# gopi-erabati/Object-Pose-Estimation

Measured on AMD Instinct MI355X. Metric: ICP iterations/sec (1M scene pts vs 100k model pts) at 1/2/4/8 GPU, higher is better.
Workload: dtype f32

## Files before the change

### object-pose-estimation_amd/csrc/api.hip

```cpp
#include <algorithm>
#include <cfloat>
#include <cmath>
#include <cstring>
#include <limits>
#include <numeric>

#include <chrono>
#include <thread>

#include "ope_internal.hpp"
#include "stage_host.hpp"

namespace ope {

static thread_local std::string g_global_err;

constexpr double kGridMaxTreeShare = 0.03, kGridMinTreeShare = 0.015;
constexpr size_t kGridMinQueries = 0;
constexpr float kHeavyLoadFactor = 1.0f;
constexpr float kHeavyLoadFactorStatic = 1.5f;
constexpr float kHeavyMaxChunksPerWave = 1.8f;

int set_err(ope_ctx *ctx, int code, const std::string &msg) {
  if (ctx) ctx->err = msg;
// ... 179 lines not shown
  if (ctx->grid_auto && grid_probe_poll(ctx, it_done) > 0) {
    const int rcs = switch_kernel(ctx, true, it_done, nch);
    if (rcs != OPE_OK) return rcs;
    --ctx->acc_launches;
    return enqueue_accumulate(ctx, atomic_sums);
  }
  if (ctx->plan_pending) {
    OPE_HIP(ctx, hipStreamWaitEvent(ctx->stream, ctx->ev_plan_done, 0));
    ctx->plan_cur ^= 1;
    ctx->plan_cur_slots = ctx->plan_pending_slots;
    ctx->plan_valid = true;
    ctx->plan_pending = false;
  }
  const bool plan_step = !no_plan && nch > 1 && it_done >= 1 && plan_step_after(ctx, it_done);
  if (plan_step) {
    const float chunks_per_wave = (float)nch / (float)(ctx->n_cu * 4 * kAccWavesPerSimd);
    const float heavy_factor = chunks_per_wave > kHeavyMaxChunksPerWave ? 0.0f : std::min(7.0f, std::max(2.0f, 1.2f + 1.5f * chunks_per_wave));
    const bool static_deal = ctx->cert_run && ctx->cert_seen && ctx->run_params.corr_mode == OPE_CORR_NEAREST && !ctx->run_params.use_reciprocal;
    const float load_factor = chunks_per_wave > kHeavyMaxChunksPerWave ? (static_deal ? kHeavyLoadFactorStatic : kHeavyLoadFactor) : 0.0f;
    hipStream_t ps = ctx->plan_stream;
    const int nxt = ctx->plan_cur ^ 1;
    OPE_HIP(ctx, hipEventRecord(ctx->ev_acc_done, ctx->stream));
    OPE_HIP(ctx, hipStreamWaitEvent(ps, ctx->ev_acc_done, 0));
    if (ctx->grid_auto && it_done >= 8) {
      const int rcp = grid_probe_issue(ctx, ps);
      if (rcp != OPE_OK) return rcp;
    }
    size_t tb = ctx->plan_tmp_bytes;
    if (chunk_plan(ps, cost_r, ctx->d_plan_sorted[nxt], ctx->d_chunk_ids, ctx->d_plan_order[nxt], nch, ctx->d_plan_tmp, tb) != 0)
      return set_err(ctx, OPE_EHIP, "chunk plan sort failed");
    uint32_t *out = ctx->d_plan_out + 8 * nxt;
    const uint32_t group_slots = static_deal ? 8u : (uint32_t)kFrontLanes;
    const float slot_share = static_deal ? kOctSlotShare : kFrontSlotShare;
    plan_heavy(ps, ctx->d_plan_sorted[nxt], nch, heavy_factor, load_factor, (uint32_t)ctx->acc_blocks * (kAccBlock / 64), group_slots, slot_share, out);
    const bool slots = ctx->run_params.corr_mode == OPE_CORR_NEAREST && !ctx->run_params.use_reciprocal;
    if (slots) plan_slots(ps, ctx->d_plan_sorted[nxt], nch, out, group_slots, slot_share, ctx->d_plan_slots[nxt]);
    OPE_HIP(ctx, hipEventRecord(ctx->ev_plan_done, ps));
    ctx->plan_pending = true;
    ctx->plan_pending_slots = slots;
  }
  const ope_icp_params &p = ctx->run_params;
  const bool nrm = p.corr_mode == OPE_CORR_NORMAL_SHOOTING || p.use_surface_normal_rej || p.use_self_occluded_rej ||
                   p.estimator == OPE_EST_POINT_TO_PLANE_LLS;
  const bool recip = p.use_reciprocal != 0;
  const uint32_t packet_min = (uint32_t)ctx->n_cu * 4u * (uint32_t)kAccWavesPerSimd;
  const bool packet = p.tree_walk == OPE_WALK_PACKET ? (ctx->run_tgt->d_axis2 != nullptr && p.corr_mode == OPE_CORR_NEAREST && !recip)
                      : p.tree_walk == OPE_WALK_LANE ? false : nch > packet_min;
  ++ctx->kernel_launches[p.corr_mode != OPE_CORR_NEAREST ? OPE_KERNEL_KNN : (packet && !recip) ? OPE_KERNEL_TREE_PACKET : OPE_KERNEL_TREE_LANE];
  const bool certify = ctx->cert_run && ctx->cert_seen && p.corr_mode == OPE_CORR_NEAREST && !recip;
  AccTreeLaunch a;
  fill_acc_launch(ctx, a, certify, cost_w, atomic_sums);
  a.nrm = nrm;
  a.chunk_order = ctx->plan_valid ? ctx->d_plan_order[ctx->plan_cur] : nullptr;
  a.mode = p.corr_mode;
  a.recip = recip;
  a.srcix = recip ? ctx->run_src_index->view() : ctx->run_tgt->view();
  a.work_counter = ctx->d_work_counter;
  a.packet = packet;
  a.k_normal_shooting = p.k_normal_shooting;
  a.slot_list = (ctx->plan_valid && ctx->plan_cur_slots) ? ctx->d_plan_slots[ctx->plan_cur] : nullptr;
  a.knn_rk = p.corr_mode == OPE_CORR_NORMAL_SHOOTING ? ctx->d_knn_rk : nullptr;
  a.plan_out = ctx->d_plan_out + 8 * ctx->plan_cur;
  a.deal = ctx->d_deal;
  a.deal_parity = ctx->deal_parity;
  launch_icp_accumulate(a);
  ctx->deal_parity ^= 1u;
  return OPE_OK;
// ... 1397 lines not shown
```

### object-pose-estimation_amd/csrc/icp_kernels.hip

```cpp
#include <cstdlib>
#include <hip/hip_ext.h>

#include "bvh_traverse.hpp"
#include "lm_solve.hpp"
#include "icp_update.hpp"

namespace ope {

typedef const __attribute__((address_space(3))) float *lds_cfloat_ptr;
static_assert(kCertCand >= 1 && kCertCand <= 8, "skip certificates: candidates per query");

__device__ __forceinline__ uint32_t chain_load(const uint32_t *p) { return __hip_atomic_load(p, __ATOMIC_RELAXED, __HIP_MEMORY_SCOPE_AGENT); }
__device__ __forceinline__ void chain_store(uint32_t *p, uint32_t v) { __hip_atomic_store(p, v, __ATOMIC_RELAXED, __HIP_MEMORY_SCOPE_AGENT); }
__device__ __forceinline__ void chain_wait_own_memory_ops() { __builtin_amdgcn_s_waitcnt(0); }
__device__ __forceinline__ bool acc_launch_begin(const IcpState *st, uint32_t *chain, uint32_t chain_seq, float *s_const, uint32_t wait_ticks) {
  if (chain == nullptr) return st->done == 0;
  __shared__ uint32_t s_go[2];
  if (threadIdx.x == 0) {
    uint32_t go = 1u;
    const unsigned long long t0 = wall_clock64();
    while ((int32_t)(chain_load(chain + 1) - chain_seq) < 0) {
      if (wall_clock64() - t0 > (unsigned long long)wait_ticks) { go = 0u; atomicOr(chain + 2, 1u); break; }
      __builtin_amdgcn_s_sleep(2);
    }
    s_go[0] = go;
  }
  __syncthreads();
  if (threadIdx.x < 12) s_const[threadIdx.x] = __hip_atomic_load(&st->Ff[threadIdx.x], __ATOMIC_RELAXED, __HIP_MEMORY_SCOPE_AGENT);
  else if (threadIdx.x == 12) s_go[1] = (uint32_t)__hip_atomic_load(&st->done, __ATOMIC_RELAXED, __HIP_MEMORY_SCOPE_AGENT);
  else if (threadIdx.x == 17) s_const[17] = __hip_atomic_load(&st->last_move, __ATOMIC_RELAXED, __HIP_MEMORY_SCOPE_AGENT);
  __syncthreads();
  return s_go[0] != 0u && s_go[1] == 0u;
}
__device__ __forceinline__ void acc_launch_end(uint32_t *chain) {
  if (chain == nullptr) return;
  chain_wait_own_memory_ops();
  __syncthreads();
  if (threadIdx.x == 0) __hip_atomic_fetch_add(chain, 1u, __ATOMIC_RELAXED, __HIP_MEMORY_SCOPE_AGENT);
}

__device__ __forceinline__ uint32_t deal_pop(uint32_t *counters, uint32_t stripe, uint32_t lane_id) {
  uint32_t k = 0u;
  if (lane_id == 0u) k = __hip_atomic_fetch_add(counters + stripe * kDealLineWords, 1u, __ATOMIC_RELAXED, __HIP_MEMORY_SCOPE_AGENT);
  return k;
}
constexpr uint32_t kDealNone = 0xffffffffu;
__device__ __forceinline__ uint32_t deal_next(uint32_t k, uint32_t stripe, uint32_t n_stripes, uint32_t n_waves, uint32_t n_slots) {
  const uint32_t slot = n_waves + stripe + k * n_stripes;
  return slot < n_slots ? slot : kDealNone;
}
__device__ __forceinline__ void deal_clear_other_set(uint32_t *deal, uint32_t parity) {
  if (blockIdx.x == 0 && threadIdx.x < kDealStripes)
    __hip_atomic_store(deal + (size_t)(parity ^ 1u) * kDealStripes * kDealLineWords + threadIdx.x * kDealLineWords, 0u, __ATOMIC_RELAXED, __HIP_MEMORY_SCOPE_AGENT);
}

template <bool NRM>
__device__ __forceinline__ void add_query_sums(double *acc, lds_cfloat_ptr cs2, uint32_t lane_id, bool ok, bool p2p, float x, float y, float z,
                                               const float4 t, const float4 tn, float d2) {
    {
      asm volatile("" : "+v"(cs2));
      const float psx = cs2[12], psy = cs2[13], psz = cs2[14];
      const double sx = (double)x - (double)psx, sy = (double)y - (double)psy, sz = (double)z - (double)psz;
      const double tx = (double)t.x - (double)psx, ty = (double)t.y - (double)psy, tz = (double)t.z - (double)psz;
      const double w = ok ? 1.0 : 0.0;
      double term[kNumSums];
      term[0] = w;
      term[1] = w * sx; term[2] = w * sy; term[3] = w * sz;
      term[4] = w * tx; term[5] = w * ty; term[6] = w * tz;
      term[7] = w * (tx * sx); term[8] = w * (tx * sy); term[9] = w * (tx * sz);
      term[10] = w * (ty * sx); term[11] = w * (ty * sy); term[12] = w * (ty * sz);
      term[13] = w * (tz * sx); term[14] = w * (tz * sy); term[15] = w * (tz * sz);
      term[16] = ok ? (double)d2 : 0.0;
#pragma unroll
      for (int k = 0; k < kNumSums; ++k) {
        const double r = row16_sum(term[k]);
        if ((lane_id & 15u) == 0u) unsafeAtomicAdd(acc + k, r);
      }
      if (NRM && p2p) {
        const float v0 = __fsub_rn(__fmul_rn(tn.z, y), __fmul_rn(tn.y, z));
        const float v1 = __fsub_rn(__fmul_rn(tn.x, z), __fmul_rn(tn.z, x));
        const float v2 = __fsub_rn(__fmul_rn(tn.y, x), __fmul_rn(tn.x, y));
        const float dd = __fsub_rn(__fsub_rn(__fsub_rn(__fadd_rn(__fadd_rn(__fmul_rn(tn.x, t.x), __fmul_rn(tn.y, t.y)), __fmul_rn(tn.z, t.z)),
                                                         __fmul_rn(tn.x, x)), __fmul_rn(tn.y, y)), __fmul_rn(tn.z, z));
        const double v[6] = {w * (double)v0, w * (double)v1, w * (double)v2, w * (double)tn.x, w * (double)tn.y, w * (double)tn.z};
        int slot = kNumSums;
#pragma unroll
// ... 113 lines not shown
  else if (threadIdx.x < 15) s_const[threadIdx.x] = (float)st->pivot[threadIdx.x - 12];
  else if (threadIdx.x == 15) s_const[15] = best0;
  else if (threadIdx.x == 17) { if (chain == nullptr) s_const[17] = st->last_move; }
  else if (threadIdx.x == 30) s_ncert = 0u;
  __syncthreads();
  if (MODE == 2 && knn_rk != nullptr && blockIdx.x == 0 && threadIdx.x == 0) const_cast<IcpState *>(st)->knn_acc_flag = 1;
  constexpr bool cert_on = CERT;
  if (cert_on && threadIdx.x == 0) {
    s_const[18] = st->cert_k;
    s_const[19] = st->cert_cap;
    if (blockIdx.x == 0) atomicAdd(work_counter + 42, 1u);
  }
  if (cert_on) __syncthreads();
  const bool rej_sn = NRM && st->use_surface_normal_rej;
  const bool rej_so = NRM && st->use_self_occluded_rej;
  const bool store_pos = st->estimator == OPE_EST_POINT_TO_PLANE_LM;
  const double thr_sn = st->surface_normal_thr, thr_so = st->self_occluded_thr;
  const double max_dist_unsq = st->max_corr_dist;
  const int kk = st->k_normal_shooting;

  if ((threadIdx.x & 63u) < (uint32_t)kNumSumsMax) s_red[threadIdx.x >> 6][threadIdx.x & 63u] = 0.0;
  const bool p2p = NRM && st->estimator == OPE_EST_POINT_TO_PLANE_LLS;

  const uint32_t lane_id = threadIdx.x & 63u;
  const uint32_t n_waves = gridDim.x * (BLOCK / 64);
  const uint32_t wave_id = (uint32_t)__builtin_amdgcn_readfirstlane((int)(blockIdx.x * (BLOCK / 64) + (threadIdx.x >> 6)));
  const uint32_t n_chunks = (src.n_valid + 63u) / 64u;
  const bool measuring = chunk_order && measuring_launch != 0u;
  const uint32_t n_heavy = (OCT_OK && chunk_order && !measuring) ? min(plan_out[0], n_chunks) : 0u;
  constexpr uint32_t GW = CERT ? 8u : (uint32_t)kFrontLanes;
  const bool listed = OCT_OK && slot_list != nullptr && chunk_order != nullptr && !measuring && n_heavy > 0u && plan_out[6] == GW;
  const uint32_t n_slots = n_chunks + (GW - 1u) * n_heavy;
  const bool dealt = chunk_order != nullptr && !CERT;
  uint32_t *const deal_set = deal + (size_t)deal_parity * kDealStripes * kDealLineWords;
  const uint32_t n_stripes = min(kDealStripes, n_waves);
  const uint32_t stripe = wave_id % n_stripes;
  const uint32_t n_alone = (dealt || !chunk_order) ? 0u
                           : listed             ? min(plan_out[7], n_waves / 2u)
                                                : min(min(plan_out[5] + (measuring ? min(plan_out[0], n_chunks) : 0u), n_chunks - n_heavy), n_waves / 2u);
  const uint32_t n_snake = n_slots - n_alone, snake_waves = n_waves - n_alone;
  auto static_slot = [&](uint32_t r) -> uint32_t {
    if (wave_id < n_alone) return r == 0u ? (listed ? wave_id : GW * n_heavy + wave_id) : kDealNone;
    const uint32_t w = wave_id - n_alone;
    const uint32_t sn = r * snake_waves + ((r & 1u) ? (snake_waves - 1u - w) : w);
    if (sn >= n_snake) return kDealNone;
    return (listed || sn >= GW * n_heavy) ? sn + n_alone : sn;
  };
  uint32_t round = 0u;
  uint32_t slot = static_slot(0u);
  while (slot != kDealNone) {
    uint32_t ticket_v = 0u;
    bool oct;
    uint32_t ord, sub;
    if (listed) {
      const uint32_t e = slot_list[slot];
      oct = (e >> 31) != 0u;
      sub = (e >> 28) & 7u;
      ord = e & 0x0fffffffu;
    } else {
      oct = slot < GW * n_heavy;
      ord = oct ? (slot / GW) : (n_heavy + (slot - GW * n_heavy));
      sub = slot % GW;
    }
    const uint32_t chunk = chunk_order ? chunk_order[ord] : ord;
    const uint32_t base = chunk * 64u;
    const unsigned long long t_begin = __builtin_amdgcn_s_memtime();
    const uint32_t i = oct ? (base + sub * (64u / GW) + (lane_id / GW)) : (base + lane_id);
    const bool active = i < src.n_valid;
    const bool owner = active && (!oct || (lane_id & (GW - 1u)) == 0u);
    lds_cfloat_ptr cst = (lds_cfloat_ptr)s_const;
    asm volatile("" : "+v"(cst));
    float F[12];
#pragma unroll
    for (int k = 0; k < 12; ++k) F[k] = cst[k];
    const float4 s = src.xyzw[active ? i : base];
    const float x = xform_row(F + 0, s.x, s.y, s.z);
    const float y = xform_row(F + 4, s.x, s.y, s.z);
    const float z = xform_row(F + 8, s.x, s.y, s.z);
    float nx = 0.f, ny = 0.f, nz = 0.f;
    if (NRM && src.nrm != nullptr) {
      const float4 n4 = src.nrm[active ? i : base];
      nx = rot_row(F + 0, n4.x, n4.y, n4.z);
      ny = rot_row(F + 4, n4.x, n4.y, n4.z);
      nz = rot_row(F + 8, n4.x, n4.y, n4.z);
    }
    bool ok;
    float d2;
    uint32_t pos = 0;
    int match = -1;
    if constexpr (CERT) {
      const float best_init = active ? cst[15] : -INFINITY;
      const size_t cstride = src.n;
      bool need = active, stuck = false, has_cert = false;
      float c_best = INFINITY;
      uint32_t c_pos = 0u;
      if (active) need = !cert_check(tgt, cert_q, cert_l, cert_pos, cstride, i, x, y, z, best_init, cst[17], c_best, c_pos, stuck, has_cert);
      const bool build = need && !stuck && owner && cert_worth_building(corr_d2[i], cst[18], cst[19], cst[17]);
      const uint32_t h = need ? hint[i] : 0u;
      if (dealt) ticket_v = deal_pop(deal_set, stripe, lane_id);
      const bool fast = need && !build && !(oct && __shfl((int)build, (int)(lane_id & ~7u), 64) != 0);
      NearestVisitor v{fast ? best_init : -INFINITY, kNoPos, 0};
      const unsigned long long fmask = __ballot(fast);
      if (fmask != 0ull) {
        if (oct) {
          if (fast) bvh_traverse_oct(tgt, x, y, z, v, &s_stk[0][threadIdx.x & ~7u], BLOCK, h);
        } else if (__popcll(fmask) <= 8) {
          const uint32_t r = lane_id >> 3;
          const bool serve = r < (uint32_t)__popcll(fmask);
          unsigned long long mm = fmask;
          for (uint32_t k = 0; k < r && mm != 0ull; ++k) mm &= mm - 1ull;
          const int from = mm != 0ull ? (int)__builtin_ctzll(mm) : 0;
          const float gx = __shfl(x, from, 64), gy = __shfl(y, from, 64), gz = __shfl(z, from, 64);
          const uint32_t gh = (uint32_t)__shfl((int)h, from, 64);
          NearestVisitor gv{serve ? cst[15] : -INFINITY, kNoPos, 0};
          if (serve) bvh_traverse_oct(tgt, gx, gy, gz, gv, &s_stk[0][threadIdx.x & ~7u], BLOCK, gh);
          const int back = 8 * (int)__popcll(fmask & ((1ull << lane_id) - 1ull));
          const float rb = __shfl(gv.best, back, 64);
          const uint32_t rp = (uint32_t)__shfl((int)gv.pos, back, 64), rl = (uint32_t)__shfl((int)gv.leaf, back, 64);
          if (fast) { v.best = rb; v.pos = rp; v.leaf = rl; }
        } else {
          const bool done = PACKET && bvh_traverse_packet(tgt, x, y, z, fast, v, h, stk, BLOCK);
          if (!done && fast) bvh_traverse_deferred(tgt, x, y, z, v, stk, BLOCK, h, min(8, kMaxDepth + 1 - tgt.depth));
        }
      }
      float r_best = fast ? v.best : c_best;
      uint32_t r_pos = fast ? v.pos : c_pos, r_leaf = fast ? v.leaf : h;
      if (__ballot(build) != 0ull) cert_build(tgt, cert_q, cert_l, cert_pos, cstride, i, x, y, z, best_init, h, stk, BLOCK, build, build, r_best, r_pos, r_leaf);
      {
        const uint32_t nc = (uint32_t)__popcll(__ballot(owner && !need));
        if (lane_id == 0 && nc != 0u) atomicAdd(&s_ncert, nc);
      }
      if (owner && r_leaf != h) hint[i] = r_leaf;
      const bool found = active && r_pos != kNoPos;
      pos = found ? r_pos : 0;
      ok = found && !((double)r_best > max_d2);
      d2 = found ? r_best : INFINITY;
      match = found ? (store_pos ? (int)pos : __float_as_int(tgt.pts[pos].w)) : -1;
    } else if constexpr (MODE == 0) {
      NearestVisitor v{active ? cst[15] : -INFINITY, kNoPos, 0};
      const uint32_t h = active ? hint[i] : 0u;
      if (dealt) ticket_v = deal_pop(deal_set, stripe, lane_id);
      if (OCT_OK && oct) {
        if (active) bvh_traverse_front<kFrontLanes>(tgt, x, y, z, v, &s_stk[0][threadIdx.x & ~(GW - 1u)], BLOCK, h);
      } else {
        const bool done = PACKET && bvh_traverse_packet(tgt, x, y, z, active, v, h, stk, BLOCK);
        if (!done && active) bvh_traverse_deferred(tgt, x, y, z, v, stk, BLOCK, h, min(8, kMaxDepth + 1 - tgt.depth));
      }
      if (owner && v.leaf != h) hint[i] = v.leaf;
      const bool found = active && v.pos != kNoPos;
      ok = found && !((double)v.best > max_d2);
      d2 = found ? v.best : INFINITY;
      pos = found ? v.pos : 0;
      match = found ? (store_pos ? (int)pos : __float_as_int(tgt.pts[pos].w)) : -1;
      if (RECIP) {
        float G[12];
#pragma unroll
        for (int k = 0; k < 12; ++k) G[k] = st->Finv[k];
        const float4 t = tgt.pts[pos];
        const float bx = xform_row(G + 0, t.x, t.y, t.z), by = xform_row(G + 4, t.x, t.y, t.z), bz = xform_row(G + 8, t.x, t.y, t.z);
        NearestVisitor r{ok ? cst[15] : -INFINITY, kNoPos, 0};
        if (ok) bvh_traverse(srcix, bx, by, bz, r, stk, BLOCK);
        ok = ok && r.pos != kNoPos && !((double)r.best > max_d2) &&
             __float_as_int(srcix.pts[r.pos].w) == __float_as_int(s.w);
      }
    } else if constexpr (MODE == 2) {
      constexpr int K = KREG;
      KnnRegVisitor<K> v;
      float bound0 = INFINITY;
      if (knn_rk != nullptr && active && st->have_prev) {
        const float rk = knn_rk[i];
        if (rk < 3.0e38f) {
          const float ox = xform_row(st->Fprev + 0, s.x, s.y, s.z), oy = xform_row(st->Fprev + 4, s.x, s.y, s.z), oz = xform_row(st->Fprev + 8, s.x, s.y, s.z);
          const float delta = sqrtf(sq_dist3(x - ox, y - oy, z - oz));
          const float b = sqrtf(rk) * 1.00001f + delta * 1.00001f + 1e-6f * (fabsf(x) + fabsf(y) + fabsf(z)) + 1e-30f;
          bound0 = b * b * 1.00001f;
        }
      }
      const uint32_t h0 = active ? hint[i] : 0u;
      if (dealt) ticket_v = deal_pop(deal_set, stripe, lane_id);
      bool todo = active;
      for (;;) {
        if (todo) {
          v.init(true, bound0);
          bvh_traverse(tgt, x, y, z, v, stk, BLOCK, h0);
        }
        const bool retry = todo && bound0 < 3.0e38f && v.count < K;
        if (__ballot(retry) == 0ull) break;
        todo = retry;
        bound0 = INFINITY;
      }
      if (!active) v.init(false);
      if (active) {
        hint[i] = v.leaf;
        if (knn_rk != nullptr) knn_rk[i] = v.count >= K ? v.d[K - 1] : INFINITY;
      }
      double min_dist = 1.79769313486231570815e308;
      d2 = INFINITY;
      pos = 0;
#pragma unroll
      for (int j = 0; j < K; ++j) {
        if (j < v.count && j < kk) {
          const float4 p = tgt.pts[v.p[j]];
          const double vx = (double)__fsub_rn(p.x, x), vy = (double)__fsub_rn(p.y, y), vz = (double)__fsub_rn(p.z, z);
          const double cx = (double)ny * vz - (double)nz * vy;
          const double cy = (double)nz * vx - (double)nx * vz;
          const double cz = (double)nx * vy - (double)ny * vx;
          const double dist = cx * cx + cy * cy + cz * cz;
          if (dist < min_dist) { min_dist = dist; d2 = v.d[j]; pos = v.p[j]; }
        }
      }
      ok = active && v.count > 0 && !(min_dist > max_dist_unsq);
      match = v.count > 0 ? (store_pos ? (int)pos : __float_as_int(tgt.pts[pos].w)) : -1;
    } else {
      if (dealt) ticket_v = deal_pop(deal_set, stripe, lane_id);
      float *ld = reinterpret_cast<float *>(s_dyn) + threadIdx.x;
      uint32_t *lp = reinterpret_cast<uint32_t *>(s_dyn + sizeof(float) * BLOCK * kKnnMaxK) + threadIdx.x;
      KnnVisitor v{ld, lp, BLOCK, kk, 0, active ? INFINITY : -INFINITY};
      bvh_traverse(tgt, x, y, z, v, stk, BLOCK);
      double min_dist = 1.79769313486231570815e308;
      int min_j = 0;
      for (int j = 0; j < v.count; ++j) {
        const float4 p = tgt.pts[lp[j * BLOCK]];
        const double vx = (double)__fsub_rn(p.x, x), vy = (double)__fsub_rn(p.y, y), vz = (double)__fsub_rn(p.z, z);
        const double cx = (double)ny * vz - (double)nz * vy;
        const double cy = (double)nz * vx - (double)nx * vz;
        const double cz = (double)nx * vy - (double)ny * vx;
        const double dist = cx * cx + cy * cy + cz * cz;
        if (dist < min_dist) { min_dist = dist; min_j = j; }
      }
      ok = active && v.count > 0 && !(min_dist > max_dist_unsq);
      d2 = v.count > 0 ? ld[min_j * BLOCK] : INFINITY;
      pos = v.count > 0 ? lp[min_j * BLOCK] : 0;
      match = v.count > 0 ? (store_pos ? (int)pos : __float_as_int(tgt.pts[pos].w)) : -1;
    }
    if (NRM && ok && rej_sn) {
      const float4 tn = tgt.nrm[pos];
      const float score = __fadd_rn(__fadd_rn(__fmul_rn(nx, tn.x), __fmul_rn(ny, tn.y)), __fmul_rn(nz, tn.z));
      ok = (double)score > thr_sn;
    }
    if (NRM && ok && rej_so) {
      const double sl = sqrt((double)__fadd_rn(__fadd_rn(__fmul_rn(x, x), __fmul_rn(y, y)), __fmul_rn(z, z)));
      const double score = (double)nx * (-(double)x / sl) + (double)ny * (-(double)y / sl) + (double)nz * (-(double)z / sl);
      ok = score > thr_so;
    }
    ok = ok && owner;
    if (owner) {
      __builtin_nontemporal_store(ok ? match : -1, corr_match + i);
      __builtin_nontemporal_store(d2, corr_d2 + i);
    }
    add_query_sums<NRM>(s_red[threadIdx.x >> 6], (lds_cfloat_ptr)s_const, lane_id, ok, p2p, x, y, z, tgt.pts[ok ? pos : 0],
                        (NRM && p2p) ? tgt.nrm[ok ? pos : 0] : make_float4(0.f, 0.f, 0.f, 0.f), d2);
    if (lane_id == 0 && !oct) chunk_cost[chunk] = (uint32_t)((__builtin_amdgcn_s_memtime() - t_begin) >> 4);
    if (dealt) {
      slot = deal_next((uint32_t)__builtin_amdgcn_readfirstlane((int)ticket_v), stripe, n_stripes, n_waves, n_slots);
    } else {
      slot = static_slot(++round);
    }
  }

  __syncthreads();
  if (threadIdx.x < (p2p ? kNumSumsMax : kNumSums)) {
    double v = 0.0;
#pragma unroll
    for (int w = 0; w < BLOCK / 64; ++w) v += s_red[w][threadIdx.x];
    if (S_atomic != nullptr) unsafeAtomicAdd(S_atomic + threadIdx.x, v);
    else partials[threadIdx.x * kAccMaxBlocks + blockIdx.x] = v;
  }
  if (CERT && threadIdx.x == 64 && s_ncert != 0u)
    atomicAdd(reinterpret_cast<unsigned long long *>(work_counter + 40), (unsigned long long)s_ncert);
  acc_launch_end(chain);
}

constexpr int kGridMaxSpan = 3;
constexpr int kGridRowBatch = 4;

__device__ __forceinline__ void grid_axis_range(float c, float r, float lo, float inv, int dim, int &a, int &b) {
  a = min(max((int)floorf(__fmul_rn(__fsub_rn(__fsub_rn(c, r), lo), inv)), 0), dim - 1);
  b = min(max((int)floorf(__fmul_rn(__fsub_rn(__fadd_rn(c, r), lo), inv)), 0), dim - 1);
}

__device__ __forceinline__ bool grid_scan(const GridView &g, float qx, float qy, float qz, float &best, uint32_t &gpos) {
  const float r = __fadd_rn(__fmul_rn(__fsqrt_rn(best), 1.0005f), g.eps);
  int ax, bx, ay, by, az, bz;
  grid_axis_range(qx, r, g.lo[0], g.inv, g.dim[0], ax, bx);
  grid_axis_range(qy, r, g.lo[1], g.inv, g.dim[1], ay, by);
  grid_axis_range(qz, r, g.lo[2], g.inv, g.dim[2], az, bz);
  const int ny = by - ay + 1, nz = bz - az + 1, nrow = ny * nz;
// ... 748 lines not shown
```

### object-pose-estimation_amd/csrc/ope_internal.hpp

```cpp
#pragma once

#include <hip/hip_runtime.h>

#include <algorithm>
#include <atomic>
#include <cstdint>
#include <memory>
#include <mutex>
#include <string>
#include <unordered_map>
#include <utility>
#include <cstdio>
#include <cstdlib>
#include <cstring>
#include <vector>

#include "../../include/ope.h"

namespace ope {

constexpr int kNodeFloats = 12;
constexpr int kMaxDepth = 20;
constexpr size_t kPtsPad = 8;

// ... 42 lines not shown
  double surface_normal_thr, self_occluded_thr;
  long long n_corr;
  int max_iterations, failure_after_max_iter, min_correspondences;
  int iterations, converged, state, done;
  int corr_mode, k_normal_shooting, use_surface_normal_rej, use_self_occluded_rej, use_reciprocal, estimator;
  int comm_error;
  int chain_error;
  float Fprev[12];
  int have_prev;
  int knn_acc_flag;
  int cert_mode;
  float cert_thr;
  float cert_cap;
  float cert_k;
  float src_c[3];
  float src_r;
  float last_move;
  uint32_t *host_cert;
};
static_assert(sizeof(IcpState) % 8 == 0, "IcpState holds doubles");

constexpr int kP2pMaxRanks = 8;
constexpr int kP2pMaxSums = 96;
constexpr int kP2pSlotWords = 2 * kP2pMaxSums;
constexpr size_t kP2pBufferBytes = sizeof(unsigned long long) * 2 * kP2pMaxRanks * kP2pSlotWords;
struct P2pView {
  unsigned long long *buf[kP2pMaxRanks];
  int nranks, rank;
};

constexpr float kOctSlotShare = 0.42f;
constexpr int kFrontLanes = 4;
constexpr float kFrontSlotShare = 0.55f;
constexpr float kCertWorth = 24.0f;
constexpr int kCertCand = 5;
constexpr int kNumSums = 17;
constexpr int kNumSumsMax = 44;
constexpr int kAccBlock = 512;
constexpr int kAccWavesPerSimd = 6;
constexpr int kAccMaxBlocks = 1024;
constexpr uint32_t kDealStripes = 64;
constexpr uint32_t kDealLineWords = 32;
constexpr size_t kDealBytes = sizeof(uint32_t) * 2 * kDealStripes * kDealLineWords;

struct GrejWork;

}

template <class T>
struct default_init_allocator : std::allocator<T> {
  template <class U> struct rebind { using other = default_init_allocator<U>; };
  using std::allocator<T>::allocator;
  template <class U, class... Args> void construct(U *p, Args &&...args) {
    if constexpr (sizeof...(Args) == 0) ::new (static_cast<void *>(p)) U;
    else ::new (static_cast<void *>(p)) U(std::forward<Args>(args)...);
  }
};

struct ope_ctx {
  int device = -1;
  int n_cu = 256;
  int n_xcd = 8;
  uint32_t wait_ticks = 200000000u;
  hipStream_t own_stream = nullptr;
  hipStream_t stream = nullptr;
  std::string err;

  ope::IcpState *d_state = nullptr;
  double *d_partials = nullptr;
  double *d_lm_stats = nullptr;
  uint32_t *d_work_counter = nullptr;
  int32_t *d_corr_match = nullptr;
  float *d_corr_d2 = nullptr;
  uint32_t *d_chunk_cost = nullptr, *d_chunk_cost_sorted = nullptr, *d_chunk_ids = nullptr, *d_chunk_order = nullptr;
  uint32_t *d_slot_list = nullptr;
  bool slot_list_valid = false;
// ... 445 lines not shown
struct AccGridLaunch : AccLaunch {
  GridView grid{};
  uint32_t *ghint = nullptr, *cert_stats = nullptr;
  const uint32_t *qorder = nullptr;
  unsigned char *qclass = nullptr;
};
void launch_icp_accumulate(const AccTreeLaunch &a);
void launch_icp_accumulate_grid(const AccGridLaunch &a);
int icp_accumulate_blocks_per_cu(bool nrm, bool packet, bool grid);
int icp_accumulate_cert_blocks_per_cu(bool nrm, bool packet, bool grid);
void launch_icp_reduce_update(hipStream_t stream, IcpState *st, const double *partials, double *S, int nblocks, bool do_update,
                              uint32_t *work_counter);
void launch_icp_p2p_update(hipStream_t stream, IcpState *st, double *S, int nsums, const P2pView &pv, uint32_t seq,
                           unsigned long long timeout_ticks, bool do_update, double *out_sums);
void launch_icp_lm_update(hipStream_t stream, IcpState *st, double *S, double *stats);
void launch_icp_update_chained(hipStream_t stream, IcpState *st, int nsums, uint32_t *chain, uint32_t seq, uint32_t tickets, uint32_t wait_ticks);
void launch_icp_update(hipStream_t stream, IcpState *st, double *S, int nsums, const float *Tk_ext);
void launch_gather_fixed_pairs(hipStream_t stream, const CloudView &src, const CloudView &tgt, const uint32_t *pos, uint32_t n, float4 *fix);
void launch_icp_fixed_pairs(hipStream_t stream, const IcpState *st, const float4 *fix, uint32_t n, double *S, float2 *seen);
void launch_pairs_svd(hipStream_t stream, const float *d_src, const float *d_tgt, uint32_t n, double *d_partials, int nblocks, float *d_out_T);
void launch_nn_search(hipStream_t stream, const CloudView &q, const BvhView &tgt, const float *d_T, int32_t *out_idx, float *out_d2);
void launch_knn_search(hipStream_t stream, const CloudView &q, const BvhView &tgt, const float *d_T, int k, int32_t *out_idx, float *out_d2);
void launch_seed_hints(hipStream_t stream, const CloudView &src, const BvhView &tgt, const IcpState *st, uint32_t *hint);
void launch_fitness(hipStream_t stream, int nblocks, const CloudView &q, const BvhView &tgt, const float *d_T, double max_range,
                    double *partials, const uint32_t *hint);
void launch_lm_pos_to_orig(hipStream_t stream, const BvhView &tgt, int32_t *d_corr, uint32_t n);
void launch_lm_stats(hipStream_t stream, int n_cu, const CloudView &src, const BvhView &tgt, const IcpState *st, const int32_t *d_corr_pos,
                     double *d_stats);
int chunk_plan(hipStream_t stream, const uint32_t *cost, uint32_t *cost_sorted, const uint32_t *ids, uint32_t *order, uint32_t n, void *tmp,
               size_t &tmp_bytes);
void plan_slots(hipStream_t stream, const uint32_t *cost_sorted_desc, uint32_t n, const uint32_t *plan_info, uint32_t slots, float share,
                uint32_t *slot_list);
void plan_heavy(hipStream_t stream, const uint32_t *cost_sorted_desc, uint32_t n, float factor, float load_factor, uint32_t n_waves,
                uint32_t slots, float share, uint32_t *plan_info);
void grid_count_far(hipStream_t stream, const float *corr_d2, uint32_t n_valid, float thr2, uint32_t *plan_info);
int grid_plan(hipStream_t stream, bool repartition, const unsigned char *qclass, uint32_t n_valid, uint32_t *qorder, uint32_t *plan_info,
              const uint32_t *cost, uint32_t *keys, uint32_t *cost_sorted, const uint32_t *ids, uint32_t *order, uint32_t nch, uint32_t n_waves,
              float factor_override, float load_factor, void *tmp, size_t tmp_bytes);
size_t grid_plan_tmp_bytes(uint32_t n_valid, uint32_t nch);
void fill_iota(hipStream_t stream, uint32_t *v, uint32_t n);
hipError_t concat_device(hipStream_t stream, const CloudView &a, const float *d_T_rows, const CloudView &b, float *d_raw, float lo[3],
                         float hi[3], const uint32_t *rgb_a, const uint32_t *rgb_b, uint32_t *d_rgb_raw);
hipError_t build_bvh_device(hipStream_t stream, const float4 *d_src, const float4 *d_src_nrm, size_t n, int leaf_size, const float bb_lo[3],
                            const float bb_hi[3], int *out_depth, float4 **d_nodes, float4 **d_pts, float4 **d_nrm, float4 **d_axis2,
                            bool tmp_alloc);
hipError_t build_grid_device(hipStream_t stream, const float4 *d_pts, const float4 *d_nrm, size_t n_, const float bb_lo[3],
                             const float bb_hi[3], double fill_target, uint32_t max_cells, GridView *out, float4 **out_gpts, float4 **out_gnrm,
                             uint32_t **out_cell_start, uint32_t **out_gpos);
void grid_hints_to_leaves(hipStream_t stream, const uint32_t *ghint, const uint32_t *gpos_of_bvhpos, uint32_t nq, uint32_t n_t, int depth,
                          uint32_t *hint, uint32_t *d_inv);
void grid_count_outside(hipStream_t stream, const CloudView &src, const float rows[12], const float lo[3], const float hi[3], float margin,
                        uint32_t *d_count);
int comm_allreduce_sums(ope_ctx *ctx, double *d_sums, int count);
bool comm_uses_p2p(const ope_ctx *ctx);
int comm_p2p_exchange_update(ope_ctx *ctx, IcpState *d_state, double *d_sums, int nsums);
int comm_p2p_exchange(ope_ctx *ctx, double *d_sums, int nsums);

}
```

### object-pose-estimation_amd/csrc/sampling.hip

```cpp
#include <cstring>
#include <string>

#include <algorithm>
#include <rocprim/rocprim.hpp>

#include <cfloat>
#include <cmath>
#include <vector>

#include "morton.hpp"
#include "ope_internal.hpp"

namespace ope {

__global__ __launch_bounds__(256) void voxel_key_kernel(CloudView c, float inv_leaf, int min_bx, int min_by, int min_bz,
                                                         unsigned div_x, unsigned div_xy, int idx_bits, unsigned long long *keys,
                                                         uint32_t *vals) {
  const uint32_t i = blockIdx.x * 256 + threadIdx.x;
  if (i >= c.n) return;
  vals[i] = i;
  if (i >= c.n_valid) { keys[i] = ~0ull; return; }
  const float4 p = c.xyzw[i];
  const int ix = (int)floorf(p.x * inv_leaf) - min_bx, iy = (int)floorf(p.y * inv_leaf) - min_by,
            iz = (int)floorf(p.z * inv_leaf) - min_bz;
  const unsigned long long voxel = (unsigned long long)ix + (unsigned long long)iy * div_x + (unsigned long long)iz * div_xy;
  keys[i] = (voxel << idx_bits) | (unsigned long long)(uint32_t)__float_as_int(p.w);
}

__global__ __launch_bounds__(256) void voxel_min_kernel(CloudView c, float inv_leaf, const unsigned long long *__restrict__ keys,
                                                         const uint32_t *__restrict__ vals, uint32_t n_valid, int idx_bits,
                                                         unsigned long long *__restrict__ best) {
  const uint32_t p = blockIdx.x * 256 + threadIdx.x;
  const uint32_t lane = threadIdx.x & 63u;
  const bool on = p < n_valid;
  unsigned long long vox = ~0ull, m = ~0ull;
  if (on) {
    vox = keys[p] >> idx_bits;
    const float4 q = c.xyzw[vals[p]];
    const float ix = floorf(q.x * inv_leaf), iy = floorf(q.y * inv_leaf), iz = floorf(q.z * inv_leaf);
    const float d = (q.x - ix) * (q.x - ix) + (q.y - iy) * (q.y - iy) + (q.z - iz) * (q.z - iz) + 1.0f;
    m = ((unsigned long long)__float_as_uint(d) << 32) | (unsigned long long)p;
  }
// ... 35 lines not shown
  if (i < n) v[i] = i;
}

int chunk_plan(hipStream_t stream, const uint32_t *cost, uint32_t *cost_sorted, const uint32_t *ids, uint32_t *order,
               uint32_t n, void *tmp, size_t &tmp_bytes) {
  hipError_t e = rocprim::radix_sort_pairs_desc(tmp, tmp_bytes, cost, cost_sorted, ids, order, n, 0, 32, stream);
  return e == hipSuccess ? 0 : -1;
}

__device__ __forceinline__ uint32_t count_costlier(const uint32_t *cost_sorted_desc, uint32_t cap, float thr) {
  uint32_t lo = 0, hi = cap;
  while (lo < hi) {
    const uint32_t mid = (lo + hi) / 2;
    if ((float)cost_sorted_desc[mid] > thr) lo = mid + 1; else hi = mid;
  }
  return lo;
}

__host__ __device__ constexpr double group_work(uint32_t slots, float share) { return (double)slots * (double)share; }
constexpr double kOctWork = group_work(8u, kOctSlotShare);
__device__ __forceinline__ double block_sum_range(const uint32_t *v, uint32_t a, uint32_t b, double *s_sum) {
  double acc = 0.0;
  for (uint32_t i = a + threadIdx.x; i < b; i += 256) acc += (double)v[i];
  __syncthreads();
  s_sum[threadIdx.x] = acc;
  __syncthreads();
  for (int off = 128; off >= 1; off >>= 1) {
    if ((int)threadIdx.x < off) s_sum[threadIdx.x] += s_sum[threadIdx.x + off];
    __syncthreads();
  }
  return s_sum[0];
}
__global__ __launch_bounds__(1024) void plan_heavy_kernel(const uint32_t *cost_sorted_desc, uint32_t n, float factor, float load_factor,
                                                          uint32_t n_waves, uint32_t slots, float share, uint32_t *plan_info) {
  using scan_t = rocprim::block_scan<double, 1024>;
  __shared__ typename scan_t::storage_type scan_storage;
  __shared__ double s_pre[1024];
  const uint32_t per = (n + 1023u) / 1024u;
  double acc = 0.0;
  for (uint32_t i = threadIdx.x * per; i < min(n, (threadIdx.x + 1u) * per); ++i) acc += (double)cost_sorted_desc[i];
  double excl = 0.0;
  scan_t().exclusive_scan(acc, excl, 0.0, scan_storage);
  s_pre[threadIdx.x] = excl;
  __syncthreads();
  if (threadIdx.x != 0) return;
  auto sum_first = [&](uint32_t m) {
    m = min(m, n);
    const uint32_t blk = per ? min(m / per, 1023u) : 0u;
    double v = s_pre[blk];
    for (uint32_t i = blk * per; i < m; ++i) v += (double)cost_sorted_desc[i];
    return v;
  };
  const double total = sum_first(n);
  uint32_t nh = 0, k = 0;
  double rest = total;
  if (n >= 8) {
    if (factor > 0.f) nh = count_costlier(cost_sorted_desc, n / 4, factor * (float)cost_sorted_desc[n / 2]);
    else if (load_factor > 0.f) nh = count_costlier(cost_sorted_desc, n / 4, load_factor * (float)(total / (double)max(n_waves, 1u)));
  }
  const double heavy = sum_first(nh);
  const double gwork = group_work(slots, share);
  rest = gwork * heavy + (total - heavy);
  for (int pass = 0; pass < 4; ++pass) {
    const uint32_t w_left = n_waves > k ? n_waves - k : 1u;
    const float fair = (float)(rest / (double)w_left);
    uint32_t lo = nh, hi = min(n, nh + n_waves / 2u);
    while (lo < hi) {
      const uint32_t mid = (lo + hi) / 2;
      if ((float)cost_sorted_desc[mid] >= fair && fair > 0.f) lo = mid + 1; else hi = mid;
    }
    const uint32_t k_new = lo - nh;
    if (k_new == k) break;
    k = k_new;
    rest = gwork * heavy + (total - heavy) - (sum_first(nh + k) - heavy);
  }
  plan_info[0] = nh;
  plan_info[5] = k;
  plan_info[6] = slots;
  const uint32_t w_left = n_waves > k ? n_waves - k : 1u;
  const float fair = (float)(rest / (double)w_left);
  uint32_t lo = 0, hi = nh;
  while (lo < hi) {
    const uint32_t mid = (lo + hi) / 2;
    if (share * (float)cost_sorted_desc[mid] >= fair && fair > 0.f) lo = mid + 1; else hi = mid;
  }
  plan_info[7] = min(k + slots * lo, n_waves / 2u);
}

__global__ __launch_bounds__(256) void plan_slots_kernel(const uint32_t *__restrict__ cost_sorted_desc, uint32_t n, const uint32_t *__restrict__ plan_info,
                                                         uint32_t slots, float share, uint32_t *__restrict__ slot_list) {
  const uint32_t r = blockIdx.x * 256 + threadIdx.x;
  if (r >= n) return;
  const uint32_t nh = min(plan_info[0], n);
  const float c = (float)cost_sorted_desc[r];
  if (r < nh) {
    const float key = share * c;
    uint32_t lo = nh, hi = n;
    while (lo < hi) {
      const uint32_t mid = (lo + hi) / 2;
      if ((float)cost_sorted_desc[mid] >= key) lo = mid + 1; else hi = mid;
    }
    const uint32_t base = slots * r + (lo - nh);
    for (uint32_t j = 0; j < slots; ++j) slot_list[base + j] = r | (j << 28) | 0x80000000u;
  } else {
    uint32_t lo = 0, hi = nh;
    while (lo < hi) {
      const uint32_t mid = (lo + hi) / 2;
      if (share * (float)cost_sorted_desc[mid] > c) lo = mid + 1; else hi = mid;
    }
    slot_list[(r - nh) + slots * lo] = r;
  }
}

void plan_slots(hipStream_t stream, const uint32_t *cost_sorted_desc, uint32_t n, const uint32_t *plan_info, uint32_t slots, float share,
                uint32_t *slot_list) {
  hipLaunchKernelGGL(plan_slots_kernel, dim3((n + 255) / 256), dim3(256), 0, stream, cost_sorted_desc, n, plan_info, slots, share, slot_list);
}

void plan_heavy(hipStream_t stream, const uint32_t *cost_sorted_desc, uint32_t n, float factor, float load_factor, uint32_t n_waves,
                uint32_t slots, float share, uint32_t *plan_info) {
  hipLaunchKernelGGL(plan_heavy_kernel, dim3(1), dim3(1024), 0, stream, cost_sorted_desc, n, factor, load_factor, n_waves, slots, share, plan_info);
}

__global__ void grid_plan_keys_kernel(const uint32_t *__restrict__ cost, uint32_t nch, uint32_t n_valid, const uint32_t *__restrict__ plan_info,
                                      uint32_t *__restrict__ keys) {
  const uint32_t c = blockIdx.x * 256 + threadIdx.x;
  if (c >= nch) return;
  const uint32_t n_tc = (n_valid - min(plan_info[1], n_valid) + 63u) / 64u;
  keys[c] = c < n_tc ? max(cost[c], 1u) : 0u;
}

__global__ __launch_bounds__(256) void grid_plan_heavy_kernel(const uint32_t *cost_sorted_desc, const uint32_t *cost, uint32_t n_valid, uint32_t n_waves,
                                                              float factor_override, float load_factor, uint32_t *plan_info) {
  __shared__ double s_sum[256];
  __shared__ uint32_t s_nh, s_k;
  const uint32_t n = (n_valid - min(plan_info[1], n_valid) + 63u) / 64u;
  const uint32_t n_gc = (min(plan_info[1], n_valid) + 63u) / 64u;
  const double tree_total = block_sum_range(cost_sorted_desc, 0, n, s_sum);
  const double grid_total = block_sum_range(cost, n, n + n_gc, s_sum);
  const double total = tree_total + grid_total;
  if (threadIdx.x == 0) {
    const float cpw = (float)n / (float)max(n_waves, 1u);
    const float factor = factor_override >= 0.f ? factor_override : fminf(7.0f, fmaxf(2.0f, 1.2f + 1.5f * cpw));
    const float load = (8.0f * (float)n + 0.33f * (float)n_gc) / (float)max(n_waves, 1u);
    uint32_t nh = 0;
    if (n >= 8) {
      if (factor_override >= 0.f || load <= 1.8f) { if (factor > 0.f) nh = count_costlier(cost_sorted_desc, n / 4, factor * (float)cost_sorted_desc[n / 2]); }
      else if (load_factor > 0.f) nh = count_costlier(cost_sorted_desc, n / 4, load_factor * (float)(total / (double)max(n_waves, 1u)));
    }
    s_nh = nh;
    s_k = 0;
  }
  __syncthreads();
  const uint32_t nh = s_nh;
// ... 487 lines not shown
```

Measured before the change: 17080.

## Split dealt work queue into two regions served by separate wave roles

Splits the dynamic deal queue in the accumulate kernel into a front and a far region, each with its own striped atomic counters. Half the waves in each block draw from each region and switch to the other region once their own is exhausted. The split point is computed in the planning kernel by a cost-weighted search. The aim is to cut contention on the deal counters and improve tail balance, at the cost of more planning work, extra counter memory, and LDS bookkeeping. The planning kernel's prefix-sum loop is also unrolled by 8.

After: 17460, median of 6. +2.3%, better.

```diff
diff --git a/object-pose-estimation_amd/csrc/api.hip b/object-pose-estimation_amd/csrc/api.hip
--- a/object-pose-estimation_amd/csrc/api.hip
+++ b/object-pose-estimation_amd/csrc/api.hip
@@ -235,7 +235,8 @@
     uint32_t *out = ctx->d_plan_out + 8 * nxt;
     const uint32_t group_slots = static_deal ? 8u : (uint32_t)kFrontLanes;
     const float slot_share = static_deal ? kOctSlotShare : kFrontSlotShare;
-    plan_heavy(ps, ctx->d_plan_sorted[nxt], nch, heavy_factor, load_factor, (uint32_t)ctx->acc_blocks * (kAccBlock / 64), group_slots, slot_share, out);
+    plan_heavy(ps, ctx->d_plan_sorted[nxt], nch, heavy_factor, load_factor, (uint32_t)ctx->acc_blocks * (kAccBlock / 64), group_slots, slot_share,
+               static_deal ? 0.0f : kFarRegionShare , out);
     const bool slots = ctx->run_params.corr_mode == OPE_CORR_NEAREST && !ctx->run_params.use_reciprocal;
     if (slots) plan_slots(ps, ctx->d_plan_sorted[nxt], nch, out, group_slots, slot_share, ctx->d_plan_slots[nxt]);
     OPE_HIP(ctx, hipEventRecord(ctx->ev_plan_done, ps));
diff --git a/object-pose-estimation_amd/csrc/deal_queue.hpp b/object-pose-estimation_amd/csrc/deal_queue.hpp
--- /dev/null
+++ b/object-pose-estimation_amd/csrc/deal_queue.hpp
@@ -0,0 +1,91 @@
+#pragma once
+#include <cstdint>
+
+#if defined(__HIPCC__) || defined(__CUDACC__)
+#define OPE_DQ_HD __host__ __device__ inline
+#else
+#define OPE_DQ_HD inline
+#endif
+
+namespace ope {
+
+constexpr uint32_t kDealNone = 0xffffffffu;
+constexpr uint32_t kDealRoleWaves = 4u;
+
+struct DealSpan {
+  uint32_t first;
+  uint32_t end;
+};
+OPE_DQ_HD uint32_t deal_entry(DealSpan s, uint32_t k, uint32_t n_stripes) {
+  const uint32_t pos = s.first + k * n_stripes;
+  return pos < s.end ? pos : kDealNone;
+}
+OPE_DQ_HD DealSpan deal_whole(uint32_t stripe, uint32_t n_waves, uint32_t n_slots) { return DealSpan{n_waves + stripe, n_slots}; }
+
+OPE_DQ_HD uint32_t deal_role(uint32_t wave_in_block) { return wave_in_block >= kDealRoleWaves ? 1u : 0u; }
+OPE_DQ_HD uint32_t deal_role_rank(uint32_t block, uint32_t wave_in_block) { return block * kDealRoleWaves + (wave_in_block & (kDealRoleWaves - 1u)); }
+OPE_DQ_HD bool deal_two_regions(bool dealt, uint32_t split, uint32_t n_slots, uint32_t n_waves) {
+  return dealt && split > 0u && split < n_slots && n_slots > n_waves;
+}
+OPE_DQ_HD uint32_t deal_region_begin(uint32_t region, uint32_t split) { return region ? split : 0u; }
+OPE_DQ_HD uint32_t deal_region_end(uint32_t region, uint32_t split, uint32_t n_slots) { return region ? n_slots : split; }
+OPE_DQ_HD uint32_t deal_region_first(uint32_t region, uint32_t rank, uint32_t split, uint32_t n_slots) {
+  const uint32_t pos = deal_region_begin(region, split) + rank;
+  return pos < deal_region_end(region, split, n_slots) ? pos : kDealNone;
+}
+OPE_DQ_HD DealSpan deal_region(uint32_t region, uint32_t stripe, uint32_t n_role, uint32_t split, uint32_t n_slots) {
+  return DealSpan{deal_region_begin(region, split) + n_role + stripe, deal_region_end(region, split, n_slots)};
+}
+OPE_DQ_HD DealSpan deal_other_region(DealSpan own, uint32_t role, uint32_t split, uint32_t n_slots) {
+  return role ? DealSpan{own.first - split, split} : DealSpan{own.first + split, n_slots};
+}
+
+template <class SumFirst>
+OPE_DQ_HD uint32_t deal_split(const uint32_t *c, uint32_t n, uint32_t nh, uint32_t slots, float share, float rho, SumFirst sum_first) {
+  const double w = (double)slots * (double)share;
+  const double heavy = sum_first(nh), total = sum_first(n);
+  const double all = w * heavy + (total - heavy);
+  const double target = all * ((double)rho / (1.0 + (double)rho));
+  if (!(target > 0.0)) return 0u;
+  auto groups_before = [&](uint32_t q, uint32_t glo, uint32_t ghi) {
+    if (q >= n) return ghi;
+    const float cq = (float)c[q];
+    while (glo < ghi) {
+      const uint32_t mid = (glo + ghi) / 2u;
+      if (share * (float)c[mid] > cq) glo = mid + 1u; else ghi = mid;
+    }
+    return glo;
+  };
+  uint32_t qlo = nh, qhi = n, glo = 0u, ghi = nh;
+  uint32_t g_prev = 0u;
+  double front_prev = -1.0;
+  uint32_t q_prev = nh;
+  while (qlo < qhi) {
+    const uint32_t mid = (qlo + qhi) / 2u;
+    const uint32_t g = groups_before(mid, glo, ghi);
+    const double front = (sum_first(mid) - heavy) + w * sum_first(g);
+    if (front >= target) { qhi = mid; ghi = g; }
+    else { qlo = mid + 1u; glo = g; g_prev = g; front_prev = front; q_prev = mid; }
+  }
+  const uint32_t q = qlo;
+  uint32_t pos = 0u;
+  double front = 0.0;
+  if (front_prev >= 0.0) {
+    pos = (q_prev - nh) + slots * g_prev + 1u;
+    front = front_prev + (double)c[q_prev];
+    if (front >= target) return pos;
+  }
+  uint32_t lo = g_prev, hi = ghi;
+  const double base = front - w * sum_first(g_prev);
+  while (lo < hi) {
+    const uint32_t mid = (lo + hi) / 2u;
+    if (base + w * sum_first(mid + 1u) >= target) hi = mid; else lo = mid + 1u;
+  }
+  if (lo >= ghi) return (q - nh) + slots * ghi;
+  const double before = base + w * sum_first(lo), one = (double)share * (double)c[lo];
+  uint32_t j = 1u;
+  while (j < slots && before + (double)j * one < target) ++j;
+  return pos + slots * (lo - g_prev) + j;
+}
+
+}
diff --git a/object-pose-estimation_amd/csrc/icp_kernels.hip b/object-pose-estimation_amd/csrc/icp_kernels.hip
--- a/object-pose-estimation_amd/csrc/icp_kernels.hip
+++ b/object-pose-estimation_amd/csrc/icp_kernels.hip
@@ -2,6 +2,7 @@
 #include <hip/hip_ext.h>
 
 #include "bvh_traverse.hpp"
+#include "deal_queue.hpp"
 #include "lm_solve.hpp"
 #include "icp_update.hpp"
 
@@ -39,19 +40,18 @@
   if (threadIdx.x == 0) __hip_atomic_fetch_add(chain, 1u, __ATOMIC_RELAXED, __HIP_MEMORY_SCOPE_AGENT);
 }
 
-__device__ __forceinline__ uint32_t deal_pop(uint32_t *counters, uint32_t stripe, uint32_t lane_id) {
+__device__ __forceinline__ uint32_t deal_pop(uint32_t *counter, uint32_t lane_id) {
   uint32_t k = 0u;
-  if (lane_id == 0u) k = __hip_atomic_fetch_add(counters + stripe * kDealLineWords, 1u, __ATOMIC_RELAXED, __HIP_MEMORY_SCOPE_AGENT);
+  if (lane_id == 0u) k = __hip_atomic_fetch_add(counter, 1u, __ATOMIC_RELAXED, __HIP_MEMORY_SCOPE_AGENT);
   return k;
 }
-constexpr uint32_t kDealNone = 0xffffffffu;
-__device__ __forceinline__ uint32_t deal_next(uint32_t k, uint32_t stripe, uint32_t n_stripes, uint32_t n_waves, uint32_t n_slots) {
-  const uint32_t slot = n_waves + stripe + k * n_stripes;
-  return slot < n_slots ? slot : kDealNone;
+__device__ __forceinline__ uint32_t *deal_counters(uint32_t *deal, uint32_t region, uint32_t parity) {
+  return deal + (size_t)(2u * region + parity) * kDealStripes * kDealLineWords;
 }
 __device__ __forceinline__ void deal_clear_other_set(uint32_t *deal, uint32_t parity) {
-  if (blockIdx.x == 0 && threadIdx.x < kDealStripes)
-    __hip_atomic_store(deal + (size_t)(parity ^ 1u) * kDealStripes * kDealLineWords + threadIdx.x * kDealLineWords, 0u, __ATOMIC_RELAXED, __HIP_MEMORY_SCOPE_AGENT);
+  if (blockIdx.x == 0 && threadIdx.x < 2u * kDealStripes)
+    __hip_atomic_store(deal_counters(deal, threadIdx.x / kDealStripes, parity ^ 1u) + (threadIdx.x % kDealStripes) * kDealLineWords, 0u, __ATOMIC_RELAXED,
+                       __HIP_MEMORY_SCOPE_AGENT);
 }
 
 template <bool NRM>
@@ -231,9 +231,35 @@
   const bool listed = OCT_OK && slot_list != nullptr && chunk_order != nullptr && !measuring && n_heavy > 0u && plan_out[6] == GW;
   const uint32_t n_slots = n_chunks + (GW - 1u) * n_heavy;
   const bool dealt = chunk_order != nullptr && !CERT;
-  uint32_t *const deal_set = deal + (size_t)deal_parity * kDealStripes * kDealLineWords;
-  const uint32_t n_stripes = min(kDealStripes, n_waves);
-  const uint32_t stripe = wave_id % n_stripes;
+  static_assert(!OCT_OK || BLOCK / 64 == 2 * (int)kDealRoleWaves, "two roles of kDealRoleWaves waves per block");
+  const uint32_t split = (OCT_OK && dealt) ? (listed ? plan_out[1] : (n_heavy == 0u ? plan_out[2] : 0u)) : 0u;
+  bool may_switch = OCT_OK && deal_two_regions(dealt, split, n_slots, n_waves);
+  const uint32_t role_rank = (uint32_t)__builtin_amdgcn_readfirstlane((int)deal_role_rank(blockIdx.x, threadIdx.x >> 6));
+  const uint32_t n_stripes = may_switch ? min(kDealStripes, n_waves / 2u) : min(kDealStripes, n_waves);
+  uint32_t *deal_ctr;
+  DealSpan span;
+  uint32_t slot0;
+  if (may_switch) {
+    const uint32_t role = (uint32_t)__builtin_amdgcn_readfirstlane((int)deal_role(threadIdx.x >> 6));
+    deal_ctr = deal_counters(deal, role, deal_parity) + (role_rank % n_stripes) * kDealLineWords;
+    span = deal_region(role, role_rank % n_stripes, n_waves / 2u, split, n_slots);
+    slot0 = deal_region_first(role, role_rank, split, n_slots);
+    if (lane_id == 0u) { s_const[16] = __uint_as_float(split); s_const[18] = __uint_as_float(n_slots); }
+  } else {
+    deal_ctr = deal_counters(deal, 0u, deal_parity) + (wave_id % n_stripes) * kDealLineWords;
+    span = deal_whole(wave_id % n_stripes, n_waves, n_slots);
+    slot0 = kDealNone;
+  }
+  auto help_other = [&]() -> uint32_t {
+    may_switch = false;
+    lds_cfloat_ptr cq = (lds_cfloat_ptr)s_const;
+    asm volatile("" : "+v"(cq));
+    const uint32_t role = (uint32_t)__builtin_amdgcn_readfirstlane((int)deal_role(threadIdx.x >> 6));
+    span = deal_other_region(span, role, (uint32_t)__builtin_amdgcn_readfirstlane(__float_as_int(cq[16])),
+                             (uint32_t)__builtin_amdgcn_readfirstlane(__float_as_int(cq[18])));
+    deal_ctr = role ? deal_ctr - 2u * kDealStripes * kDealLineWords : deal_ctr + 2u * kDealStripes * kDealLineWords;
+    return deal_entry(span, (uint32_t)__builtin_amdgcn_readfirstlane((int)deal_pop(deal_ctr, lane_id)), n_stripes);
+  };
   const uint32_t n_alone = (dealt || !chunk_order) ? 0u
                            : listed             ? min(plan_out[7], n_waves / 2u)
                                                 : min(min(plan_out[5] + (measuring ? min(plan_out[0], n_chunks) : 0u), n_chunks - n_heavy), n_waves / 2u);
@@ -246,7 +272,8 @@
     return (listed || sn >= GW * n_heavy) ? sn + n_alone : sn;
   };
   uint32_t round = 0u;
-  uint32_t slot = static_slot(0u);
+  uint32_t slot = may_switch ? slot0 : static_slot(0u);
+  if (may_switch && slot == kDealNone) slot = help_other();
   while (slot != kDealNone) {
     uint32_t ticket_v = 0u;
     bool oct;
@@ -296,7 +323,7 @@
       if (active) need = !cert_check(tgt, cert_q, cert_l, cert_pos, cstride, i, x, y, z, best_init, cst[17], c_best, c_pos, stuck, has_cert);
       const bool build = need && !stuck && owner && cert_worth_building(corr_d2[i], cst[18], cst[19], cst[17]);
       const uint32_t h = need ? hint[i] : 0u;
-      if (dealt) ticket_v = deal_pop(deal_set, stripe, lane_id);
+      if (dealt) ticket_v = deal_pop(deal_ctr, lane_id);
       const bool fast = need && !build && !(oct && __shfl((int)build, (int)(lane_id & ~7u), 64) != 0);
       NearestVisitor v{fast ? best_init : -INFINITY, kNoPos, 0};
       const unsigned long long fmask = __ballot(fast);
@@ -338,7 +365,7 @@
     } else if constexpr (MODE == 0) {
       NearestVisitor v{active ? cst[15] : -INFINITY, kNoPos, 0};
       const uint32_t h = active ? hint[i] : 0u;
-      if (dealt) ticket_v = deal_pop(deal_set, stripe, lane_id);
+      if (dealt) ticket_v = deal_pop(deal_ctr, lane_id);
       if (OCT_OK && oct) {
         if (active) bvh_traverse_front<kFrontLanes>(tgt, x, y, z, v, &s_stk[0][threadIdx.x & ~(GW - 1u)], BLOCK, h);
       } else {
@@ -376,7 +403,7 @@
         }
       }
       const uint32_t h0 = active ? hint[i] : 0u;
-      if (dealt) ticket_v = deal_pop(deal_set, stripe, lane_id);
+      if (dealt) ticket_v = deal_pop(deal_ctr, lane_id);
       bool todo = active;
       for (;;) {
         if (todo) {
@@ -411,7 +438,7 @@
       ok = active && v.count > 0 && !(min_dist > max_dist_unsq);
       match = v.count > 0 ? (store_pos ? (int)pos : __float_as_int(tgt.pts[pos].w)) : -1;
     } else {
-      if (dealt) ticket_v = deal_pop(deal_set, stripe, lane_id);
+      if (dealt) ticket_v = deal_pop(deal_ctr, lane_id);
       float *ld = reinterpret_cast<float *>(s_dyn) + threadIdx.x;
       uint32_t *lp = reinterpret_cast<uint32_t *>(s_dyn + sizeof(float) * BLOCK * kKnnMaxK) + threadIdx.x;
       KnnVisitor v{ld, lp, BLOCK, kk, 0, active ? INFINITY : -INFINITY};
@@ -451,7 +478,8 @@
                         (NRM && p2p) ? tgt.nrm[ok ? pos : 0] : make_float4(0.f, 0.f, 0.f, 0.f), d2);
     if (lane_id == 0 && !oct) chunk_cost[chunk] = (uint32_t)((__builtin_amdgcn_s_memtime() - t_begin) >> 4);
     if (dealt) {
-      slot = deal_next((uint32_t)__builtin_amdgcn_readfirstlane((int)ticket_v), stripe, n_stripes, n_waves, n_slots);
+      slot = deal_entry(span, (uint32_t)__builtin_amdgcn_readfirstlane((int)ticket_v), n_stripes);
+      if (may_switch && slot == kDealNone) slot = help_other();
     } else {
       slot = static_slot(++round);
     }
diff --git a/object-pose-estimation_amd/csrc/ope_internal.hpp b/object-pose-estimation_amd/csrc/ope_internal.hpp
--- a/object-pose-estimation_amd/csrc/ope_internal.hpp
+++ b/object-pose-estimation_amd/csrc/ope_internal.hpp
@@ -98,6 +98,7 @@
 constexpr float kOctSlotShare = 0.42f;
 constexpr int kFrontLanes = 4;
 constexpr float kFrontSlotShare = 0.55f;
+constexpr float kFarRegionShare = 0.4f;
 constexpr float kCertWorth = 24.0f;
 constexpr int kCertCand = 5;
 constexpr int kNumSums = 17;
@@ -107,7 +108,7 @@
 constexpr int kAccMaxBlocks = 1024;
 constexpr uint32_t kDealStripes = 64;
 constexpr uint32_t kDealLineWords = 32;
-constexpr size_t kDealBytes = sizeof(uint32_t) * 2 * kDealStripes * kDealLineWords;
+constexpr size_t kDealBytes = sizeof(uint32_t) * 2 * 2 * kDealStripes * kDealLineWords;
 
 struct GrejWork;
 
@@ -619,7 +620,7 @@
 void plan_slots(hipStream_t stream, const uint32_t *cost_sorted_desc, uint32_t n, const uint32_t *plan_info, uint32_t slots, float share,
                 uint32_t *slot_list);
 void plan_heavy(hipStream_t stream, const uint32_t *cost_sorted_desc, uint32_t n, float factor, float load_factor, uint32_t n_waves,
-                uint32_t slots, float share, uint32_t *plan_info);
+                uint32_t slots, float share, float far_share, uint32_t *plan_info);
 void grid_count_far(hipStream_t stream, const float *corr_d2, uint32_t n_valid, float thr2, uint32_t *plan_info);
 int grid_plan(hipStream_t stream, bool repartition, const unsigned char *qclass, uint32_t n_valid, uint32_t *qorder, uint32_t *plan_info,
               const uint32_t *cost, uint32_t *keys, uint32_t *cost_sorted, const uint32_t *ids, uint32_t *order, uint32_t nch, uint32_t n_waves,
diff --git a/object-pose-estimation_amd/csrc/sampling.hip b/object-pose-estimation_amd/csrc/sampling.hip
--- a/object-pose-estimation_amd/csrc/sampling.hip
+++ b/object-pose-estimation_amd/csrc/sampling.hip
@@ -8,6 +8,7 @@
 #include <cmath>
 #include <vector>
 
+#include "deal_queue.hpp"
 #include "morton.hpp"
 #include "ope_internal.hpp"
 
@@ -109,7 +110,7 @@
   return s_sum[0];
 }
 __global__ __launch_bounds__(1024) void plan_heavy_kernel(const uint32_t *cost_sorted_desc, uint32_t n, float factor, float load_factor,
-                                                          uint32_t n_waves, uint32_t slots, float share, uint32_t *plan_info) {
+                                                          uint32_t n_waves, uint32_t slots, float share, float far_share, uint32_t *plan_info) {
   using scan_t = rocprim::block_scan<double, 1024>;
   __shared__ typename scan_t::storage_type scan_storage;
   __shared__ double s_pre[1024];
@@ -120,14 +121,21 @@
   scan_t().exclusive_scan(acc, excl, 0.0, scan_storage);
   s_pre[threadIdx.x] = excl;
   __syncthreads();
-  if (threadIdx.x != 0) return;
   auto sum_first = [&](uint32_t m) {
     m = min(m, n);
     const uint32_t blk = per ? min(m / per, 1023u) : 0u;
     double v = s_pre[blk];
-    for (uint32_t i = blk * per; i < m; ++i) v += (double)cost_sorted_desc[i];
+    for (uint32_t i = blk * per; i < m; i += 8u) {
+      uint32_t c8[8];
+#pragma unroll
+      for (uint32_t j = 0; j < 8u; ++j) c8[j] = cost_sorted_desc[min(i + j, n - 1u)];
+#pragma unroll
+      for (uint32_t j = 0; j < 8u; ++j) v += (i + j < m) ? (double)c8[j] : 0.0;
+    }
     return v;
   };
+  if (threadIdx.x == 64u) plan_info[2] = far_share > 0.f ? deal_split(cost_sorted_desc, n, 0u, slots, share, far_share, sum_first) : 0u;
+  if (threadIdx.x != 0) return;
   const double total = sum_first(n);
   uint32_t nh = 0, k = 0;
   double rest = total;
@@ -162,6 +170,7 @@
     if (share * (float)cost_sorted_desc[mid] >= fair && fair > 0.f) lo = mid + 1; else hi = mid;
   }
   plan_info[7] = min(k + slots * lo, n_waves / 2u);
+  plan_info[1] = far_share > 0.f && nh > 0u ? deal_split(cost_sorted_desc, n, nh, slots, share, far_share, sum_first) : 0u;
 }
 
 __global__ __launch_bounds__(256) void plan_slots_kernel(const uint32_t *__restrict__ cost_sorted_desc, uint32_t n, const uint32_t *__restrict__ plan_info,
@@ -195,8 +204,8 @@
 }
 
 void plan_heavy(hipStream_t stream, const uint32_t *cost_sorted_desc, uint32_t n, float factor, float load_factor, uint32_t n_waves,
-                uint32_t slots, float share, uint32_t *plan_info) {
-  hipLaunchKernelGGL(plan_heavy_kernel, dim3(1), dim3(1024), 0, stream, cost_sorted_desc, n, factor, load_factor, n_waves, slots, share, plan_info);
+                uint32_t slots, float share, float far_share, uint32_t *plan_info) {
+  hipLaunchKernelGGL(plan_heavy_kernel, dim3(1), dim3(1024), 0, stream, cost_sorted_desc, n, factor, load_factor, n_waves, slots, share, far_share, plan_info);
 }
 
 __global__ void grid_plan_keys_kernel(const uint32_t *__restrict__ cost, uint32_t nch, uint32_t n_valid, const uint32_t *__restrict__ plan_info,
```
